# GuillaumeHolley/BloomFilterTrie

Measured on AMD Instinct MI355X. Metric: M k-mers/sec queried (presenceNode), higher is better.
Workload: dtype u64

## Files before the change

### bloomfiltertrie_amd/csrc/bft_gpu.hip

```cpp
#include <hip/hip_runtime.h>

#include <algorithm>
#include <chrono>
#include <cstring>
#include <mutex>
#include <string>
#include <vector>

#include "../../include/bft_gpu.h"
#include "bft_color_plan.h"
#include "bft_handle.h"
#include "bft_hash.h"
#include "bft_index.h"
#include "bft_run_plan.h"
#include "bft_sort.h"
#include "bft_walk.h"

#define BFT_BLOCK 256
#define BFT_ABSENT_ROW 0xFFFFFFFFu
#define BFT_MAX_GENOME_ID (1u << 24)

static thread_local std::string g_err;
int bft_fail(int code, const std::string& msg) {
    g_err = msg;
// ... 759 lines not shown
    } else if (nm == "tune") {
        if (value != 0 && h->built) {
            ENTER(h);
            CK(bft_wait_foreign_stream(h));
            HIPCK(hipStreamSynchronize(h->stream));
            CK(bft_ensure_table(h));
            CK(bft_tune_residency(h));
        }
    } else if (nm == "query_dynamic") {
        h->opt_query_dynamic = value != 0;
    } else if (nm == "query_dynamic_min") {
        h->opt_query_dynamic_min = value;
    } else if (nm == "query_chunk") {
        if (value < 1 || value > 64) return fail(BFT_GPU_E_ARG, "query_chunk must be in [1,64]");
        h->opt_query_chunk = (uint32_t)value;
    } else if (nm == "query_grid_mult") {
        if (value < 1 || value > 64) return fail(BFT_GPU_E_ARG, "query_grid_mult must be in [1,64]");
        h->opt_grid_mult = (int)value;
#if defined(BFT_PERF_PROBE)
    } else if (nm == "debug_stop") {
        h->im.debug_stop = (uint32_t)value;
#endif
    } else if (nm == "test_front_rank_mode") {
        if (value > 2) return fail(BFT_GPU_E_ARG, "test_front_rank_mode must be 0, 1 or 2");
        bft_test_front_rank_mode((int)value);
    } else if (nm == "test_front_wave_cap") {
        if (value != 0 && value != 512 && value != 1024) return fail(BFT_GPU_E_ARG, "test_front_wave_cap must be 0, 512 or 1024");
        bft_test_front_wave_cap((uint32_t)value);
    } else if (nm == "test_weak_signature") {
        if (value < 0 || value > 2) return fail(BFT_GPU_E_ARG, "test_weak_signature must be 0, 1 or 2");
// ... 108 lines not shown
```

### bloomfiltertrie_amd/csrc/bft_handle.h

```cpp
#pragma once
#include <hip/hip_runtime.h>

#include "bft_derive.h"
#include "bft_dev.h"
#include "bft_image.h"
#include "bft_ingest.h"
#include "bft_kh.h"

struct HandleScratch {
    explicit HandleScratch(const char* w) : what(w) {}
    HandleScratch(const HandleScratch&) = delete;
    HandleScratch& operator=(const HandleScratch&) = delete;
    ~HandleScratch() { if (ev) (void)hipEventDestroy(ev); }
    int acquire(hipStream_t s, bool capturing_) {
        if (used && stream != s) {
            if (capturing_) return bft_fail(BFT_GPU_E_ARG, std::string(what) + " recorded into a graph: the handle's scratch is in use on another stream");
            HIPCK(ev ? hipEventSynchronize(ev) : hipDeviceSynchronize());
            used = false;
        }
        idle = !used;
        used = true;
        stream = s;
        capturing = capturing_;
        return 0;
// ... 141 lines not shown
    uint64_t idx_sizes[9] = {0};
    int opt_wgs_per_cu = 0;
    int tuned_wgs = 0;
    int opt_probe = 0;
    int tuned_probe = 0;
    double tune_ms[3] = {0, 0, 0};
    int opt_grid_mult = 1;
    uint32_t opt_test_walk_grid = 0;
    int opt_query_dynamic = 1;
    uint64_t opt_query_dynamic_min = (uint64_t)1 << 16;
    uint32_t opt_query_chunk = 4;
    ClaimSlots claims;

    HandleScratch sq{"sequence query"};
    DevBuf sq_codes, sq_bad, sq_npos, sq_poff, sq_tmp, sq_cs, sq_tile;
    HandleScratch qc{"colour query"};
    DevBuf qc_cs, qc_tmp;
    DevBuf qc_kh;
    HandleScratch pm{"prefix query"};
    DevBuf pm_buf, pm_tmp;
    uint64_t pm_n = 0;
    HandleScratch sp{"simple paths"};
    DevBuf sp_buf, sp_tmp;
    uint64_t sp_m = 0;
    HandleScratch cc{"components"};
    DevBuf cc_buf, cc_tmp;
    uint64_t cc_m = 0, cc_sets = 0;
    HandleScratch pg{"k-mer classes"};
    DevBuf pg_buf, pg_tmp;
    uint64_t pg_m = 0, pg_sets = 0;
// ... 88 lines not shown
```

### bloomfiltertrie_amd/csrc/bft_hosttest.cpp

```cpp
#include <algorithm>
#include <cstring>
#include <string>
#include <vector>

#include "bft_hash.h"
#include "bft_index.h"
#include "bft_walk.h"
#include "bft_kh_host.h"

struct HostTrie {
    int k, L, W, B;
    std::vector<uint32_t> hashmod;
    std::vector<uint64_t> tk;
    std::vector<uint32_t> tcol, cs_off, cs_ids;
    std::vector<uint64_t> rdir, nph;
    BftKhHostTable kh;
    std::vector<uint32_t> rstart, rq, rspec;
    uint64_t rstart_plain = 0;
    BftHostIndex idx;
    BftImage im;
};

template <int W>
static void to_tform(const uint8_t* packed, uint64_t n, int B, int L, std::vector<uint64_t>& out) {
// ... 635 lines not shown
extern "C" uint64_t bft_hosttest_read_genome(void* fv, int g, uint8_t* out) {
    BftFileContent* fc = (BftFileContent*)fv;
    const std::vector<uint8_t>& v = fc->per_genome[g];
    if (out && !v.empty()) memcpy(out, v.data(), v.size());
    return v.size();
}
extern "C" void bft_hosttest_read_free(void* fv) { delete (BftFileContent*)fv; }

extern "C" int bft_hosttest_annot_encode(const uint32_t* ids, uint32_t n, uint8_t* out, uint32_t cap) {
    std::vector<uint8_t> enc;
    bft_annot_encode(ids, n, enc);
    if (enc.size() > cap) return -1;
    memcpy(out, enc.data(), enc.size());
    return (int)enc.size();
}
```

### bloomfiltertrie_amd/csrc/bft_kernels_seq.h

```cpp
#pragma once
#include "bft_kernels_seqenc.h"
#include "bft_kernels_seqwin.h"

template <int W, int BLOCK, bool STAGED, int PROBE>
__device__ __forceinline__ void seq_walk_body(const BftImage& im, const uint64_t* __restrict__ codes, const uint32_t* __restrict__ bad,
                                              const uint64_t* __restrict__ seq_off, const uint64_t* __restrict__ pos_off, const uint32_t* __restrict__ tile_seq,
                                              uint32_t n_seqs, int canonical, uint32_t* __restrict__ csout) {
    extern __shared__ __align__(16) uint8_t lds[];
    uint32_t* l_hm = (uint32_t*)lds;
    uint8_t* l_bf = lds + BFT_LDS_HM_BYTES;
    const BftNode root = im.nodes[0];
    const bool stage_root = STAGED && im.rdir == nullptr;
    const uint32_t bf_bytes = stage_root ? ((BFT_MODULO_HASH * (uint32_t)root.bf_wb + 15u) & ~15u) : 0u;
    BftCCX* l_cc = (BftCCX*)(l_bf + bf_bytes);
    {
        const uint4* g = (const uint4*)im.hashmod;
        uint4* l = (uint4*)l_hm;
        for (uint32_t i = threadIdx.x; i < BFT_LDS_HM_BYTES / 16; i += BLOCK) l[i] = g[i];
        if (stage_root) {
            const uint64_t* gb = (const uint64_t*)(im.bfT + (size_t)root.bf_off * 8);
            uint64_t* lb = (uint64_t*)l_bf;
            const uint32_t nb8 = (BFT_MODULO_HASH * (uint32_t)root.bf_wb) / 8;
            for (uint32_t i = threadIdx.x; i < nb8; i += BLOCK) lb[i] = gb[i];
            for (uint32_t i = threadIdx.x; i < root.ncc; i += BLOCK) l_cc[i] = im.ccx[root.cc_first + i];
// ... 20 lines not shown
}

template <int W, bool STAGED, int PROBE>
__global__ __launch_bounds__(1024) __attribute__((amdgpu_waves_per_eu(8, 8))) void k_seq_walk8(
    BftImage im, const uint64_t* __restrict__ codes, const uint32_t* __restrict__ bad, const uint64_t* __restrict__ seq_off, const uint64_t* __restrict__ pos_off,
    const uint32_t* __restrict__ tile_seq, uint32_t n_seqs, int canonical, uint32_t* __restrict__ csout) {
    seq_walk_body<W, 1024, STAGED, PROBE>(im, codes, bad, seq_off, pos_off, tile_seq, n_seqs, canonical, csout);
}
template <int W, bool STAGED, int PROBE>
__global__ __launch_bounds__(BFT_BLOCK6) __attribute__((amdgpu_waves_per_eu(6, 6))) void k_seq_walk6(
    BftImage im, const uint64_t* __restrict__ codes, const uint32_t* __restrict__ bad, const uint64_t* __restrict__ seq_off, const uint64_t* __restrict__ pos_off,
    const uint32_t* __restrict__ tile_seq, uint32_t n_seqs, int canonical, uint32_t* __restrict__ csout) {
    seq_walk_body<W, BFT_BLOCK6, STAGED, PROBE>(im, codes, bad, seq_off, pos_off, tile_seq, n_seqs, canonical, csout);
}

#define SEQ_TALLY_G 2048u
#define SEQ_TALLY_WAVES 4
__global__ __launch_bounds__(64 * SEQ_TALLY_WAVES) void k_seq_tally(const uint32_t* __restrict__ csin, const uint64_t* __restrict__ pos_off, uint32_t n_seqs,
                                                                   const uint32_t* __restrict__ cs_off, const void* __restrict__ cs_ids, uint32_t cs_w, uint32_t G,
                                                                   uint32_t rowbytes, double threshold, uint32_t win, uint8_t* __restrict__ out) {
    extern __shared__ uint32_t s_cnt[];
    const uint32_t lane = threadIdx.x & 63u, wave = threadIdx.x >> 6;
    uint32_t* cnt = s_cnt + (size_t)wave * win;
    for (uint64_t s = (uint64_t)blockIdx.x * SEQ_TALLY_WAVES + wave; s < n_seqs; s += (uint64_t)gridDim.x * SEQ_TALLY_WAVES) {
        const uint64_t pa = pos_off[s], m = pos_off[s + 1] - pa;
        const uint64_t minv = (uint64_t)(int64_t)ceil((double)m * threshold);
        for (uint32_t win0 = 0; win0 < G; win0 += win) {
            const uint32_t wn = min(win, G - win0);
            for (uint32_t j = lane; j < wn; j += 64) cnt[j] = 0;
            for (uint64_t base = 0; base < m; base += 128) {
                uint32_t cs[2], len[2], qa[2], qb[2];
                bool act[2];
#pragma unroll
                for (int u = 0; u < 2; u++) cs[u] = base + 64u * u + lane < m ? csin[pa + base + 64u * u + lane] : 0xFFFFFFFFu;
#pragma unroll
                for (int u = 0; u < 2; u++) {
                    const uint32_t pcs = __shfl_up(cs[u], 1);
                    const bool boundary = lane == 0 || pcs != cs[u];
                    const uint64_t bmask = __ballot(boundary);
                    const uint64_t above = lane == 63 ? 0ull : bmask >> (lane + 1);
                    len[u] = above ? (uint32_t)__builtin_ctzll(above) + 1u : 64u - lane;
                    act[u] = boundary && cs[u] != 0xFFFFFFFFu;
                    qa[u] = qb[u] = 0;
                }
#pragma unroll
                for (int u = 0; u < 2; u++)
                    if (act[u]) { qa[u] = cs_off[cs[u]]; qb[u] = cs_off[cs[u] + 1]; }
                uint32_t id[2][8];
#pragma unroll
                for (int u = 0; u < 2; u++) {
#pragma unroll
                    for (int j = 0; j < 8; j++) id[u][j] = act[u] && qb[u] > qa[u] ? bft_cs_id_at(cs_ids, cs_w, min(qa[u] + (uint32_t)j, qb[u] - 1u)) : 0u;
                }
#pragma unroll
                for (int u = 0; u < 2; u++) {
                    if (!act[u]) continue;
#pragma unroll
                    for (int j = 0; j < 8; j++)
                        if (qa[u] + (uint32_t)j < qb[u] && id[u][j] - win0 < wn) atomicAdd(&cnt[id[u][j] - win0], len[u]);
                    for (uint32_t q = qa[u] + 8u; q < qb[u]; q += 8) {
                        uint32_t more[8];
#pragma unroll
                        for (int j = 0; j < 8; j++) more[j] = bft_cs_id_at(cs_ids, cs_w, min(q + (uint32_t)j, qb[u] - 1u));
#pragma unroll
                        for (int j = 0; j < 8; j++)
                            if (q + (uint32_t)j < qb[u] && more[j] - win0 < wn) atomicAdd(&cnt[more[j] - win0], len[u]);
                    }
                }
            }
            __builtin_amdgcn_fence(__ATOMIC_ACQ_REL, "wavefront");
            for (uint32_t b = lane; b < (wn + 7u) / 8u; b += 64) {
                uint32_t v = 0;
                for (uint32_t j = 0; j < 8 && b * 8 + j < wn; j++) {
                    const uint32_t c = cnt[b * 8 + j];
                    if (c && c >= minv) v |= 1u << j;
                }
                out[s * rowbytes + win0 / 8 + b] = (uint8_t)v;
            }
            __builtin_amdgcn_fence(__ATOMIC_ACQ_REL, "wavefront");
        }
    }
}
```

### bloomfiltertrie_amd/csrc/bft_kernels_seqenc.h

```cpp
#pragma once
__device__ __forceinline__ int nt_code(char ch) {
    const uint32_t c = (uint8_t)ch, idx = (c & 0xDFu) - 0x41u;
    const uint32_t valid_mask = (1u << 0) | (1u << 2) | (1u << 6) | (1u << 19) | (1u << 20);
    const bool ok = idx < 21u && ((valid_mask >> idx) & 1u);
    return ok ? (int)(((c >> 1) ^ (c >> 2)) & 3u) : -1;
}

__global__ void k_seq_encode(const char* __restrict__ seqs, uint64_t n_chars, uint64_t n_words, uint64_t* __restrict__ codes, uint32_t* __restrict__ bad) {
    const bool aligned = ((uintptr_t)seqs & 15u) == 0;
    for (uint64_t wi = blockIdx.x * (uint64_t)blockDim.x + threadIdx.x; wi < n_words; wi += (uint64_t)gridDim.x * blockDim.x) {
        uint32_t d[8];
        if (aligned && wi * 32 + 32 <= n_chars) {
            const uint4* src = (const uint4*)(seqs + wi * 32);
            const uint4 a = src[0], b = src[1];
            d[0] = a.x; d[1] = a.y; d[2] = a.z; d[3] = a.w; d[4] = b.x; d[5] = b.y; d[6] = b.z; d[7] = b.w;
        } else {
#pragma unroll
            for (int j = 0; j < 8; j++) {
                uint32_t v = 0;
                for (int c = 0; c < 4; c++) {
                    const uint64_t at = wi * 32 + 4 * j + c;
                    v |= (uint32_t)(uint8_t)(at < n_chars ? seqs[at] : 'A') << (8 * c);
                }
                d[j] = v;
            }
// ... 39 lines not shown
```

### bloomfiltertrie_amd/csrc/bft_kh.h

```cpp
#pragma once
#include <hip/hip_runtime.h>
#include <stdint.h>

#include "bft_claims.h"
#include "bft_dev.h"
#include "bft_image.h"

#define BFT_KH_BLOCK 256
bool bft_kh_has_kernels(int W, uint32_t S);
struct BftKhScratch { DevBuf b[7]; };
int bft_kh_sort(const uint64_t* d_tk, const uint32_t* d_vals, uint64_t n, int k, int W, const BftKhGeo& g, BftKhScratch& sc, hipStream_t s);
int bft_kh_test_sort(int W, int shape, const uint32_t* keys, const void* recs, uint64_t n, unsigned b0, unsigned b1, uint32_t* ok, void* orec, hipStream_t s, uint32_t* h_dbase);
uint32_t bft_kh_test_sort_tile(int W, int shape);
int bft_kh_lay(uint64_t n, int k, int W, const BftKhGeo& g, uint64_t* d_kh, uint64_t* d_ovf_k, uint32_t* d_ovf_v, uint32_t* d_status, BftKhScratch& sc, hipStream_t s);
int bft_kh_dump(const BftImage& im, uint64_t* d_keys, uint64_t stride, uint32_t* d_vals, unsigned long long* d_cnt, hipStream_t s);
int bft_kh_query(const BftImage& im, int grid_mult, const uint8_t* d_kmers, uint64_t n, int rec, uint64_t* d_bits64, uint32_t* d_out32, BftClaimCtr d_ctr, uint32_t chunk,
                 hipStream_t s);
size_t bft_kh_colors_scratch_bytes(uint64_t n);
int bft_kh_color_rows(const BftImage& im, const uint8_t* d_kmers, uint64_t n, int rec, uint64_t* d_bits64, const uint8_t* bm, uint32_t stride, uint32_t rowbytes, uint8_t* d_out,
                      int device, hipStream_t s);
int bft_kh_colors(const BftImage& im, const uint8_t* d_kmers, uint64_t n, int rec, uint64_t* d_bits64, uint64_t* d_offsets, uint32_t* d_ids, uint64_t ids_cap, uint64_t* d_needed,
                  void* d_scratch, hipStream_t s);
int bft_kh_branching(const BftImage& im, const uint8_t* d_kmers, uint64_t n, int B, uint64_t* d_bits64, uint8_t* d_counts, BftClaimCtr d_ctr, uint32_t chunk, hipStream_t s);
int bft_kh_seq(const BftImage& im, const uint64_t* d_codes, const uint32_t* d_bad, const uint64_t* d_seq_off, const uint64_t* d_pos_off, const uint32_t* d_tile_seq,
               uint32_t n_seqs, int canonical, uint32_t* d_csout, BftClaimCtr d_ctr, uint32_t chunk, hipStream_t s);

int bft_walkh_query(const BftImage& im, const uint8_t* d_kmers, uint64_t n, int rec, uint64_t* d_bits64, uint32_t* d_rows, BftClaimCtr d_ctr, uint32_t grid_mult, uint32_t grid_cap, hipStream_t s);
```

### bloomfiltertrie_amd/csrc/bft_kh.hip

```cpp
#include <hip/hip_runtime.h>

#include <algorithm>
#include <atomic>
#include <cstring>

#include "bft_dev.h"
#include "bft_image.h"
#include "bft_kh.h"
#include "bft_claims.h"
#include "bft_walk.h"
#include "bft_kernels_load.h"
#include "bft_kernels_seqwin.h"
#include "bft_kh_dev.h"
#include "bft_scan.h"
#include "bft_rows16.h"
#include "bft_sort.h"

#define BFT_KH_MIN_CLAIM 4u
#define BFT_KH_MAX_CLAIM 64u
typedef BftClaims<BFT_KH_MIN_CLAIM> KhClaims;
template <int W, int S>
__global__ __launch_bounds__(BFT_KH_BLOCK) void k_query_kh(BftImage im, const uint8_t* __restrict__ packed, uint64_t n, int B, uint64_t* __restrict__ bits64,
                                                          uint32_t* __restrict__ out32, BftClaimCtr ctr, uint32_t chunk) {
    const uint64_t end_aligned = ((uint64_t)packed + n * (uint64_t)B) & ~3ull;
    const uint64_t nblk = (n + BFT_KH_BLOCK - 1) / BFT_KH_BLOCK, nwords = (n + 63) / 64;
    constexpr uint32_t WPB = BFT_KH_BLOCK / 64;
    __shared__ uint32_t s_next[2];
// ... 341 lines not shown
        const int branching = live && (cr > 1 || cl_ > 1);
        if (counts && live) counts[i] = (uint8_t)((cr << 4) | cl_);
        const uint64_t mask = __ballot(branching);
        if ((threadIdx.x & 63u) == 0) s_bits[(cl.blk - cl.start) * WPB + (threadIdx.x >> 6)] = mask;
        if (cl.last_of_round()) {
            __syncthreads();
            const uint64_t w0 = cl.start * WPB, w1 = min(nwords, cl.blk_end * WPB);
            if (w0 + threadIdx.x < w1) __builtin_nontemporal_store(s_bits[threadIdx.x], &bits64[w0 + threadIdx.x]);
        }
        cl.advance();
    }
    cl.done();
}

template <int W, int S>
__global__ __launch_bounds__(256) void k_seq_kh(BftImage im, const uint64_t* __restrict__ codes, const uint32_t* __restrict__ bad, const uint64_t* __restrict__ seq_off,
                                                const uint64_t* __restrict__ pos_off, const uint32_t* __restrict__ tile_seq, uint32_t n_seqs, int canonical,
                                                uint32_t* __restrict__ csout, BftClaimCtr ctr, uint32_t chunk) {
    const uint64_t P = pos_off[n_seqs];
    const uint64_t nblk = (P + 255) / 256;
    __shared__ uint32_t s_next[2];
    __shared__ uint4 s_lines[4][64 * BFT_KH_LDS_LINE];
    uint4* const wave_lines = s_lines[threadIdx.x >> 6];
    KhClaims cl(ctr, chunk, nblk, s_next);
    cl.first();
    for (; cl.blk < nblk; cl.advance()) {
        const uint64_t p = cl.blk * 256 + threadIdx.x;
        uint32_t cs = 0xFFFFFFFFu;
        uint64_t x[W], t[W];
        BftKhKey<W> key;
        key.home = 0; key.field = 0;
#pragma unroll
        for (int w = 0; w < W; w++) { key.body[w] = 0; key.bmask[w] = 0; }
        bool live = false;
        if (p < P) {
            uint32_t lo = tile_seq[p >> 6];
            while (lo + 1 < n_seqs && pos_off[lo + 1] <= p) lo++;
            if (seq_window<W>(codes, bad, seq_off[lo] + (p - pos_off[lo]), im.k, canonical, x)) {
                bft_tform_from_x<W>(x, im.k, t);
                bft_kh_key<W>(t, im.k, im.kh, key);
                live = true;
            }
        }
        kh_fetch_quad(im, key.home, live, wave_lines);
        if (live) {
            uint32_t val = 0;
            int res = kh_lds_scan<W, S>(im, wave_lines + (threadIdx.x & 63u) * BFT_KH_LDS_LINE, key, 0u, &val);
            for (uint32_t d = 1; res < 0 && d <= im.kh.maxd; d++) {
                const uint64_t* line = im.kh_lines + (key.home + d) * BFT_KH_LINE_WORDS;
                uint64_t hd[2];
                bft_kh_load_header(line, hd);
                res = bft_kh_scan<W, S>(im, line, hd, key, d, &val);
            }
            if (res < 0 && im.kh_ovf_n) res = bft_kh_overflow_find<W>(im, t, &val) ? 1 : 0;
            if (res > 0) cs = val;
        }
        if (p < P) csout[p] = cs;
    }
    cl.done();
}

template <int W>
struct __attribute__((packed, aligned(4))) KhRec {
    uint64_t t[W];
    uint32_t v;
};
template <int W>
struct KhSortIn {
    const uint64_t* tk;
    const uint32_t* vals;
    int k;
    BftKhGeo g;
    __device__ __forceinline__ uint32_t key(uint32_t i) const {
        uint64_t t[W];
// ... 297 lines not shown
    KH_DISPATCH(im.W, (int)im.kh.S, (kh_color_rows_launch<KW, KS>(im, d_kmers, n, rec, d_bits64, bm, stride, rowbytes, plan.tile_rows, plan.div_m, plan.div_l, d_out, device, s)));
    HIPCK(hipGetLastError());
    return 0;
}

int bft_kh_branching(const BftImage& im, const uint8_t* d_kmers, uint64_t n, int B, uint64_t* d_bits64, uint8_t* d_counts, BftClaimCtr d_ctr, uint32_t chunk, hipStream_t s) {
    const dim3 block(BFT_KH_BLOCK);
    chunk = std::max(1u, std::min(chunk, BFT_KH_BR_MAX_CLAIM));
    const dim3 grid = kh_round_grid(n, chunk, 1, d_ctr.p != nullptr);
    KH_DISPATCH(im.W, (int)im.kh.S, hipLaunchKernelGGL((k_branching_kh<KW, KS>), grid, block, 0, s, im, d_kmers, n, B, d_bits64, d_counts, d_ctr, chunk));
    HIPCK(hipGetLastError());
    return 0;
}

int bft_kh_seq(const BftImage& im, const uint64_t* d_codes, const uint32_t* d_bad, const uint64_t* d_seq_off, const uint64_t* d_pos_off, const uint32_t* d_tile_seq,
               uint32_t n_seqs, int canonical, uint32_t* d_csout, BftClaimCtr d_ctr, uint32_t chunk, hipStream_t s) {
    const dim3 grid(256 * 8), block(256);
    chunk = std::max(1u, std::min(chunk, BFT_KH_MAX_CLAIM));
    KH_DISPATCH(im.W, (int)im.kh.S,
                hipLaunchKernelGGL((k_seq_kh<KW, KS>), grid, block, 0, s, im, d_codes, d_bad, d_seq_off, d_pos_off, d_tile_seq, n_seqs, canonical, d_csout, d_ctr, chunk));
    HIPCK(hipGetLastError());
    return 0;
}
```

### bloomfiltertrie_amd/csrc/bft_query.hip

```cpp
#include <hip/hip_runtime.h>

#include <algorithm>
#include <atomic>
#include <cstring>
#include <initializer_list>
#include <type_traits>
#include <vector>

#include "bft_handle.h"
#include "bft_scan.h"
#include "bft_walk.h"

#define BFT_BLOCK 256
#define BFT_ABSENT_ROW 0xFFFFFFFFu

#include "bft_kernels_query.h"
#include "bft_kernels_seq.h"
#include "bft_kernels_color.h"

void ClaimSlots::ensure() {
    if (ctr || failed) return;
    if (hipMalloc((void**)&ctr, KH_CTR_SLOTS * 8) != hipSuccess || hipMemset(ctr, 0, KH_CTR_SLOTS * 8) != hipSuccess ||
        hipDeviceSynchronize() != hipSuccess) {
        (void)hipGetLastError();
// ... 588 lines not shown
    DevBuf dk, db, dr, dout;
    CK(dk.alloc(mc * h->B));
    CK(db.alloc(((mc + 63) / 64) * 8));
    CK(dr.alloc(mc * 4));
    CK(dout.alloc(mc * rowbytes));
    for (uint64_t a = 0; a < n; a += chunk) {
        const uint64_t m = std::min(chunk, n - a);
        CK(query_rows(h, kmers + a * h->B, m, dk, db, dr, present_bits ? present_bits + a / 8 : nullptr));
        CK(launch_color_rows(h, dr.as<uint32_t>(), m, rowbytes, dout.as<uint8_t>(), h->stream));
        HIPCK(hipMemcpyAsync(rows + a * rowbytes, dout.p, m * rowbytes, hipMemcpyDeviceToHost, h->stream));
        HIPCK(hipStreamSynchronize(h->stream));
    }
    return BFT_GPU_OK;
}

static int launch_seq_lookups(bft_gpu* h, const BftImage& image, uint32_t ns, int canonical, const uint64_t* d_soff, uint64_t units, hipStream_t s) {
    if (image.kh_lines != nullptr) {
        const ClaimSlots::Claim claim = h->claims.take(s, claims_wanted(h, h->opt_query_dynamic_min), units);
        CK(bft_kh_seq(image, h->sq_codes.as<uint64_t>(), h->sq_bad.as<uint32_t>(), d_soff, h->sq_poff.as<uint64_t>(), h->sq_tile.as<uint32_t>(), ns, canonical,
                      h->sq_cs.as<uint32_t>(), claim.ctr, h->opt_query_chunk, s));
        h->claims.launched(claim.slot, s);
        return 0;
    }
    BftImage im = image;
    im.emit_cs = 1;
    return walk_dispatch<false>(h, false, [&](auto w, auto staged, auto probe) {
        constexpr int W = decltype(w)::value, PROBE = decltype(probe)::value;
        constexpr bool STAGED = decltype(staged)::value;
        static std::atomic<uint64_t> lds_allowed{0};
        auto launch = [&](auto kernel, const WalkShape& sh) {
            CK(allow_walk_lds(lds_allowed, h->device, {(const void*)kernel}));
            hipLaunchKernelGGL(kernel, dim3(512), dim3(sh.block), sh.lds, s, im, h->sq_codes.as<uint64_t>(), h->sq_bad.as<uint32_t>(), d_soff, h->sq_poff.as<uint64_t>(),
                               h->sq_tile.as<uint32_t>(), ns, canonical, h->sq_cs.as<uint32_t>());
            HIPCK(hipGetLastError());
            return 0;
// ... 8 lines not shown
    const uint32_t G = h->im.nb_genomes, rowbytes = (G + 7) / 8;
    if (rowbytes == 0 || n_seqs == 0) return 0;
    CK(h->sq.acquire(s, bft_stream_capturing(s)));
    auto need = [&](DevBuf& b, size_t bytes) { return h->sq.grow(b, bytes, bytes / 8); };
    const uint64_t chunk = 1ull << 30;
    const uint64_t cmax = std::min(chunk, n_seqs);
    const uint64_t n_cw = (total_chars + 31) / 32;
    const size_t scan_bytes = bft_scan::scratch_bytes(cmax + 1);
    CK(need(h->sq_codes, (n_cw + BFT_MAX_W + 2) * 8));
    CK(need(h->sq_bad, (n_cw + BFT_MAX_W + 2) * 4));
    CK(need(h->sq_npos, (cmax + 1) * 8));
    CK(need(h->sq_poff, (cmax + 1) * 8));
    CK(need(h->sq_tmp, scan_bytes));
    CK(need(h->sq_tile, (total_chars / 64 + 2) * 4));
    CK(need(h->sq_cs, (total_chars + 64) * 4));
    CK(bft_zero_async(h->sq_codes.as<uint64_t>() + n_cw, (BFT_MAX_W + 2) * 8, s));
    CK(bft_zero_async(h->sq_bad.as<uint32_t>() + n_cw, (BFT_MAX_W + 2) * 4, s));
    if (n_cw)
        CK(bft_timed_launch(h, s, [&] {
            hipLaunchKernelGGL(k_seq_encode, dim3(bft_grid_for((n_cw + 255) / 256)), dim3(256), 0, s, d_seqs, total_chars, n_cw, h->sq_codes.as<uint64_t>(),
                               h->sq_bad.as<uint32_t>());
            HIPCK(hipGetLastError());
            return 0;
        }));
    for (uint64_t a = 0; a < n_seqs; a += chunk) {
        const uint64_t ns = std::min(chunk, n_seqs - a);
        const uint64_t* soff = d_seq_off + a;
        CK(bft_timed_launch(h, s, [&] {
            hipLaunchKernelGGL(k_seq_plan, dim3(bft_grid_for((ns + 256) / 256)), dim3(256), 0, s, soff, ns, h->k, h->sq_npos.as<uint64_t>());
            CK(bft_scan::exclusive_sum_ptr<uint64_t>(h->sq_npos.as<uint64_t>(), h->sq_poff.as<uint64_t>(), ns + 1, s, h->sq_tmp));
            hipLaunchKernelGGL(k_seq_tiles, dim3(256 * 4), dim3(256), 0, s, h->sq_poff.as<uint64_t>(), (uint32_t)ns, h->sq_tile.as<uint32_t>());
            HIPCK(hipGetLastError());
            return 0;
        }));
        CK(bft_timed_launch(h, s, [&] { return launch_seq_lookups(h, h->im, (uint32_t)ns, canonical, soff, total_chars / 256 + 2, s); }));
        const uint32_t win = std::min<uint32_t>(SEQ_TALLY_G, (G + 63u) & ~63u);
        CK(bft_timed_launch(h, s, [&] {
            hipLaunchKernelGGL(k_seq_tally, dim3((unsigned)std::min<uint64_t>((ns + SEQ_TALLY_WAVES - 1) / SEQ_TALLY_WAVES, 256ull * 16)), dim3(64 * SEQ_TALLY_WAVES),
                               (size_t)SEQ_TALLY_WAVES * win * 4, s, h->sq_cs.as<uint32_t>(), h->sq_poff.as<uint64_t>(), (uint32_t)ns, h->im.cs_off, h->im.cs_ids, h->im.cs_w, G,
                               rowbytes, threshold, win, d_rows + a * rowbytes);
            HIPCK(hipGetLastError());
            return 0;
        }));
    }
    h->sq.release();
    return 0;
}

extern "C" int bft_gpu_query_sequences_dev(bft_gpu* h, const void* d_seqs, const void* d_seq_off, uint64_t n_seqs, uint64_t total_chars, double threshold,
                                           int canonical, void* d_rows, void* hip_stream) {
    if (!h || ((!d_seqs || !d_seq_off || !d_rows) && n_seqs)) return bft_fail(BFT_GPU_E_ARG, "NULL argument");
    if (!(threshold > 0) || threshold > 1) return bft_fail(BFT_GPU_E_ARG, "the threshold must be in (0, 1] (reference src/bft.c:1246-1247)");
    ENTER(h);
    CK(bft_ensure_built(h, false));
    hipStream_t s = hip_stream ? (hipStream_t)hip_stream : h->stream;
// ... 59 lines not shown
```

Baseline: 52920.

## Fuse sequence k-mer lookups with colour tally for short sequences

Adds a fused k_seq_rows_kh kernel that, per group of positions, does the hash-table lookups into an LDS slice and immediately tallies colour sets into output rows. This avoids writing and re-reading the per-position colour-set buffer for short sequences. Long sequences fall back to the old lookup-then-tally kernels, which now skip short ones and exit early when no long sequences exist. The encode kernel also zeroes the slack words itself, replacing two memset launches. The change only affects sequence queries, not the measured presenceNode k-mer path.

Measured after the change: 52840. No clear change (-0.1%).

```diff
diff --git a/bloomfiltertrie_amd/csrc/bft_gpu.hip b/bloomfiltertrie_amd/csrc/bft_gpu.hip
--- a/bloomfiltertrie_amd/csrc/bft_gpu.hip
+++ b/bloomfiltertrie_amd/csrc/bft_gpu.hip
@@ -797,6 +797,9 @@
     } else if (nm == "query_chunk") {
         if (value < 1 || value > 64) return fail(BFT_GPU_E_ARG, "query_chunk must be in [1,64]");
         h->opt_query_chunk = (uint32_t)value;
+    } else if (nm == "seq_fused") {
+        if (value != 0 && value != 1) return fail(BFT_GPU_E_ARG, "seq_fused must be 0 or 1");
+        h->opt_seq_fused = (int)value;
     } else if (nm == "query_grid_mult") {
         if (value < 1 || value > 64) return fail(BFT_GPU_E_ARG, "query_grid_mult must be in [1,64]");
         h->opt_grid_mult = (int)value;
diff --git a/bloomfiltertrie_amd/csrc/bft_handle.h b/bloomfiltertrie_amd/csrc/bft_handle.h
--- a/bloomfiltertrie_amd/csrc/bft_handle.h
+++ b/bloomfiltertrie_amd/csrc/bft_handle.h
@@ -179,6 +179,8 @@
 
     HandleScratch sq{"sequence query"};
     DevBuf sq_codes, sq_bad, sq_npos, sq_poff, sq_tmp, sq_cs, sq_tile;
+    DevBuf sq_nlong;
+    int opt_seq_fused = 1;
     HandleScratch qc{"colour query"};
     DevBuf qc_cs, qc_tmp;
     DevBuf qc_kh;
diff --git a/bloomfiltertrie_amd/csrc/bft_hosttest.cpp b/bloomfiltertrie_amd/csrc/bft_hosttest.cpp
--- a/bloomfiltertrie_amd/csrc/bft_hosttest.cpp
+++ b/bloomfiltertrie_amd/csrc/bft_hosttest.cpp
@@ -7,6 +7,7 @@
 #include "bft_index.h"
 #include "bft_walk.h"
 #include "bft_kh_host.h"
+#include "bft_seq_plan.h"
 
 struct HostTrie {
     int k, L, W, B;
@@ -673,3 +674,21 @@
     memcpy(out, enc.data(), enc.size());
     return (int)enc.size();
 }
+
+extern "C" int64_t bft_hosttest_seq_plan(const uint64_t* pos_off, uint32_t n_seqs, uint64_t total_chars, uint32_t genomes, uint32_t* first_out, uint64_t cap, uint64_t* consts) {
+    const uint64_t P = pos_off[n_seqs], ntiles = (P + 63) / 64, groups = bft_seq_groups(P);
+    consts[0] = BFT_SEQ_Q; consts[1] = BFT_SEQ_C; consts[2] = BFT_SEQ_LMAX; consts[3] = BFT_SEQ_WAVES; consts[4] = groups;
+    consts[5] = bft_seq_units_bound(total_chars); consts[6] = bft_seq_lds_bytes(bft_seq_win(genomes)); consts[7] = bft_seq_win(genomes);
+    if (cap < groups + 1) return -1;
+    std::vector<uint32_t> tile_seq(ntiles + 1, 0xFFFFFFFFu);
+    for (uint64_t t = 0; t < ntiles; t++) {
+        uint32_t lo = 0, hi = n_seqs;
+        while (hi - lo > 1) {
+            const uint32_t mid = (lo + hi) >> 1;
+            if (pos_off[mid] <= t * 64) lo = mid; else hi = mid;
+        }
+        tile_seq[t] = lo;
+    }
+    for (uint64_t g = 0; g <= groups; g++) first_out[g] = bft_seq_group_first(pos_off, tile_seq.data(), n_seqs, P, g);
+    return (int64_t)groups;
+}
diff --git a/bloomfiltertrie_amd/csrc/bft_kernels_seq.h b/bloomfiltertrie_amd/csrc/bft_kernels_seq.h
--- a/bloomfiltertrie_amd/csrc/bft_kernels_seq.h
+++ b/bloomfiltertrie_amd/csrc/bft_kernels_seq.h
@@ -1,6 +1,8 @@
 #pragma once
 #include "bft_kernels_seqenc.h"
 #include "bft_kernels_seqwin.h"
+#include "bft_kernels_seqtally.h"
+#include "bft_seq_plan.h"
 
 template <int W, int BLOCK, bool STAGED, int PROBE>
 __device__ __forceinline__ void seq_walk_body(const BftImage& im, const uint64_t* __restrict__ codes, const uint32_t* __restrict__ bad,
@@ -58,70 +60,17 @@
     seq_walk_body<W, BFT_BLOCK6, STAGED, PROBE>(im, codes, bad, seq_off, pos_off, tile_seq, n_seqs, canonical, csout);
 }
 
-#define SEQ_TALLY_G 2048u
 #define SEQ_TALLY_WAVES 4
 __global__ __launch_bounds__(64 * SEQ_TALLY_WAVES) void k_seq_tally(const uint32_t* __restrict__ csin, const uint64_t* __restrict__ pos_off, uint32_t n_seqs,
                                                                    const uint32_t* __restrict__ cs_off, const void* __restrict__ cs_ids, uint32_t cs_w, uint32_t G,
-                                                                   uint32_t rowbytes, double threshold, uint32_t win, uint8_t* __restrict__ out) {
+                                                                   uint32_t rowbytes, double threshold, uint32_t win, uint8_t* __restrict__ out, const uint32_t* __restrict__ n_long) {
     extern __shared__ uint32_t s_cnt[];
+    if (n_long && *n_long == 0) return;
     const uint32_t lane = threadIdx.x & 63u, wave = threadIdx.x >> 6;
     uint32_t* cnt = s_cnt + (size_t)wave * win;
     for (uint64_t s = (uint64_t)blockIdx.x * SEQ_TALLY_WAVES + wave; s < n_seqs; s += (uint64_t)gridDim.x * SEQ_TALLY_WAVES) {
         const uint64_t pa = pos_off[s], m = pos_off[s + 1] - pa;
-        const uint64_t minv = (uint64_t)(int64_t)ceil((double)m * threshold);
-        for (uint32_t win0 = 0; win0 < G; win0 += win) {
-            const uint32_t wn = min(win, G - win0);
-            for (uint32_t j = lane; j < wn; j += 64) cnt[j] = 0;
-            for (uint64_t base = 0; base < m; base += 128) {
-                uint32_t cs[2], len[2], qa[2], qb[2];
-                bool act[2];
-#pragma unroll
-                for (int u = 0; u < 2; u++) cs[u] = base + 64u * u + lane < m ? csin[pa + base + 64u * u + lane] : 0xFFFFFFFFu;
-#pragma unroll
-                for (int u = 0; u < 2; u++) {
-                    const uint32_t pcs = __shfl_up(cs[u], 1);
-                    const bool boundary = lane == 0 || pcs != cs[u];
-                    const uint64_t bmask = __ballot(boundary);
-                    const uint64_t above = lane == 63 ? 0ull : bmask >> (lane + 1);
-                    len[u] = above ? (uint32_t)__builtin_ctzll(above) + 1u : 64u - lane;
-                    act[u] = boundary && cs[u] != 0xFFFFFFFFu;
-                    qa[u] = qb[u] = 0;
-                }
-#pragma unroll
-                for (int u = 0; u < 2; u++)
-                    if (act[u]) { qa[u] = cs_off[cs[u]]; qb[u] = cs_off[cs[u] + 1]; }
-                uint32_t id[2][8];
-#pragma unroll
-                for (int u = 0; u < 2; u++) {
-#pragma unroll
-                    for (int j = 0; j < 8; j++) id[u][j] = act[u] && qb[u] > qa[u] ? bft_cs_id_at(cs_ids, cs_w, min(qa[u] + (uint32_t)j, qb[u] - 1u)) : 0u;
-                }
-#pragma unroll
-                for (int u = 0; u < 2; u++) {
-                    if (!act[u]) continue;
-#pragma unroll
-                    for (int j = 0; j < 8; j++)
-                        if (qa[u] + (uint32_t)j < qb[u] && id[u][j] - win0 < wn) atomicAdd(&cnt[id[u][j] - win0], len[u]);
-                    for (uint32_t q = qa[u] + 8u; q < qb[u]; q += 8) {
-                        uint32_t more[8];
-#pragma unroll
-                        for (int j = 0; j < 8; j++) more[j] = bft_cs_id_at(cs_ids, cs_w, min(q + (uint32_t)j, qb[u] - 1u));
-#pragma unroll
-                        for (int j = 0; j < 8; j++)
-                            if (q + (uint32_t)j < qb[u] && more[j] - win0 < wn) atomicAdd(&cnt[more[j] - win0], len[u]);
-                    }
-                }
-            }
-            __builtin_amdgcn_fence(__ATOMIC_ACQ_REL, "wavefront");
-            for (uint32_t b = lane; b < (wn + 7u) / 8u; b += 64) {
-                uint32_t v = 0;
-                for (uint32_t j = 0; j < 8 && b * 8 + j < wn; j++) {
-                    const uint32_t c = cnt[b * 8 + j];
-                    if (c && c >= minv) v |= 1u << j;
-                }
-                out[s * rowbytes + win0 / 8 + b] = (uint8_t)v;
-            }
-            __builtin_amdgcn_fence(__ATOMIC_ACQ_REL, "wavefront");
-        }
+        if (n_long && m <= BFT_SEQ_LMAX) continue;
+        seq_tally_row([&](uint64_t j) { return csin[pa + j]; }, m, cnt, lane, cs_off, cs_ids, cs_w, G, threshold, win, out + s * rowbytes);
     }
 }
diff --git a/bloomfiltertrie_amd/csrc/bft_kernels_seqenc.h b/bloomfiltertrie_amd/csrc/bft_kernels_seqenc.h
--- a/bloomfiltertrie_amd/csrc/bft_kernels_seqenc.h
+++ b/bloomfiltertrie_amd/csrc/bft_kernels_seqenc.h
@@ -6,9 +6,15 @@
     return ok ? (int)(((c >> 1) ^ (c >> 2)) & 3u) : -1;
 }
 
+#define BFT_SEQ_SLACK_WORDS (BFT_MAX_W + 2)
 __global__ void k_seq_encode(const char* __restrict__ seqs, uint64_t n_chars, uint64_t n_words, uint64_t* __restrict__ codes, uint32_t* __restrict__ bad) {
     const bool aligned = ((uintptr_t)seqs & 15u) == 0;
-    for (uint64_t wi = blockIdx.x * (uint64_t)blockDim.x + threadIdx.x; wi < n_words; wi += (uint64_t)gridDim.x * blockDim.x) {
+    for (uint64_t wi = blockIdx.x * (uint64_t)blockDim.x + threadIdx.x; wi < n_words + BFT_SEQ_SLACK_WORDS; wi += (uint64_t)gridDim.x * blockDim.x) {
+        if (wi >= n_words) {
+            codes[wi] = 0;
+            bad[wi] = 0;
+            continue;
+        }
         uint32_t d[8];
         if (aligned && wi * 32 + 32 <= n_chars) {
             const uint4* src = (const uint4*)(seqs + wi * 32);
diff --git a/bloomfiltertrie_amd/csrc/bft_kernels_seqtally.h b/bloomfiltertrie_amd/csrc/bft_kernels_seqtally.h
--- /dev/null
+++ b/bloomfiltertrie_amd/csrc/bft_kernels_seqtally.h
@@ -0,0 +1,64 @@
+#pragma once
+#include "bft_walk.h"
+
+#define SEQ_TALLY_G 2048u
+
+template <class CsAt>
+__device__ __forceinline__ void seq_tally_row(CsAt cs_at, uint64_t m, uint32_t* cnt, uint32_t lane, const uint32_t* __restrict__ cs_off, const void* __restrict__ cs_ids,
+                                              uint32_t cs_w, uint32_t G, double threshold, uint32_t win, uint8_t* __restrict__ out_row) {
+    const uint64_t minv = (uint64_t)(int64_t)ceil((double)m * threshold);
+    for (uint32_t win0 = 0; win0 < G; win0 += win) {
+        const uint32_t wn = min(win, G - win0);
+        for (uint32_t j = lane; j < wn; j += 64) cnt[j] = 0;
+        for (uint64_t base = 0; base < m; base += 128) {
+            uint32_t cs[2], len[2], qa[2], qb[2];
+            bool act[2];
+#pragma unroll
+            for (int u = 0; u < 2; u++) cs[u] = base + 64u * u + lane < m ? cs_at(base + 64u * u + lane) : 0xFFFFFFFFu;
+#pragma unroll
+            for (int u = 0; u < 2; u++) {
+                const uint32_t pcs = __shfl_up(cs[u], 1);
+                const bool boundary = lane == 0 || pcs != cs[u];
+                const uint64_t bmask = __ballot(boundary);
+                const uint64_t above = lane == 63 ? 0ull : bmask >> (lane + 1);
+                len[u] = above ? (uint32_t)__builtin_ctzll(above) + 1u : 64u - lane;
+                act[u] = boundary && cs[u] != 0xFFFFFFFFu;
+                qa[u] = qb[u] = 0;
+            }
+#pragma unroll
+            for (int u = 0; u < 2; u++)
+                if (act[u]) { qa[u] = cs_off[cs[u]]; qb[u] = cs_off[cs[u] + 1]; }
+            uint32_t id[2][8];
+#pragma unroll
+            for (int u = 0; u < 2; u++) {
+#pragma unroll
+                for (int j = 0; j < 8; j++) id[u][j] = act[u] && qb[u] > qa[u] ? bft_cs_id_at(cs_ids, cs_w, min(qa[u] + (uint32_t)j, qb[u] - 1u)) : 0u;
+            }
+#pragma unroll
+            for (int u = 0; u < 2; u++) {
+                if (!act[u]) continue;
+#pragma unroll
+                for (int j = 0; j < 8; j++)
+                    if (qa[u] + (uint32_t)j < qb[u] && id[u][j] - win0 < wn) atomicAdd(&cnt[id[u][j] - win0], len[u]);
+                for (uint32_t q = qa[u] + 8u; q < qb[u]; q += 8) {
+                    uint32_t more[8];
+#pragma unroll
+                    for (int j = 0; j < 8; j++) more[j] = bft_cs_id_at(cs_ids, cs_w, min(q + (uint32_t)j, qb[u] - 1u));
+#pragma unroll
+                    for (int j = 0; j < 8; j++)
+                        if (q + (uint32_t)j < qb[u] && more[j] - win0 < wn) atomicAdd(&cnt[more[j] - win0], len[u]);
+                }
+            }
+        }
+        __builtin_amdgcn_fence(__ATOMIC_ACQ_REL, "wavefront");
+        for (uint32_t b = lane; b < (wn + 7u) / 8u; b += 64) {
+            uint32_t v = 0;
+            for (uint32_t j = 0; j < 8 && b * 8 + j < wn; j++) {
+                const uint32_t c = cnt[b * 8 + j];
+                if (c && c >= minv) v |= 1u << j;
+            }
+            out_row[win0 / 8 + b] = (uint8_t)v;
+        }
+        __builtin_amdgcn_fence(__ATOMIC_ACQ_REL, "wavefront");
+    }
+}
diff --git a/bloomfiltertrie_amd/csrc/bft_kh.h b/bloomfiltertrie_amd/csrc/bft_kh.h
--- a/bloomfiltertrie_amd/csrc/bft_kh.h
+++ b/bloomfiltertrie_amd/csrc/bft_kh.h
@@ -23,6 +23,9 @@
                   void* d_scratch, hipStream_t s);
 int bft_kh_branching(const BftImage& im, const uint8_t* d_kmers, uint64_t n, int B, uint64_t* d_bits64, uint8_t* d_counts, BftClaimCtr d_ctr, uint32_t chunk, hipStream_t s);
 int bft_kh_seq(const BftImage& im, const uint64_t* d_codes, const uint32_t* d_bad, const uint64_t* d_seq_off, const uint64_t* d_pos_off, const uint32_t* d_tile_seq,
-               uint32_t n_seqs, int canonical, uint32_t* d_csout, BftClaimCtr d_ctr, uint32_t chunk, hipStream_t s);
+               uint32_t n_seqs, int canonical, uint32_t* d_csout, const uint32_t* d_n_long, BftClaimCtr d_ctr, uint32_t chunk, hipStream_t s);
+int bft_kh_seq_rows(const BftImage& im, const uint64_t* d_codes, const uint32_t* d_bad, const uint64_t* d_seq_off, const uint64_t* d_pos_off, const uint32_t* d_tile_seq,
+                    uint32_t n_seqs, int canonical, double threshold, uint32_t win, uint8_t* d_rows, uint32_t* d_n_long, uint64_t units, BftClaimCtr d_ctr, uint32_t chunk, int device,
+                    hipStream_t s);
 
 int bft_walkh_query(const BftImage& im, const uint8_t* d_kmers, uint64_t n, int rec, uint64_t* d_bits64, uint32_t* d_rows, BftClaimCtr d_ctr, uint32_t grid_mult, uint32_t grid_cap, hipStream_t s);
diff --git a/bloomfiltertrie_amd/csrc/bft_kh.hip b/bloomfiltertrie_amd/csrc/bft_kh.hip
--- a/bloomfiltertrie_amd/csrc/bft_kh.hip
+++ b/bloomfiltertrie_amd/csrc/bft_kh.hip
@@ -11,6 +11,8 @@
 #include "bft_walk.h"
 #include "bft_kernels_load.h"
 #include "bft_kernels_seqwin.h"
+#include "bft_kernels_seqtally.h"
+#include "bft_seq_plan.h"
 #include "bft_kh_dev.h"
 #include "bft_scan.h"
 #include "bft_rows16.h"
@@ -382,9 +384,29 @@
 }
 
 template <int W, int S>
+__device__ __forceinline__ uint32_t kh_seq_lookup(const BftImage& im, const BftKhKey<W>& key, const uint64_t* t, bool live, uint4* wave_lines) {
+    uint32_t cs = 0xFFFFFFFFu;
+    kh_fetch_quad(im, key.home, live, wave_lines);
+    if (live) {
+        uint32_t val = 0;
+        int res = kh_lds_scan<W, S>(im, wave_lines + (threadIdx.x & 63u) * BFT_KH_LDS_LINE, key, 0u, &val);
+        for (uint32_t d = 1; res < 0 && d <= im.kh.maxd; d++) {
+            const uint64_t* line = im.kh_lines + (key.home + d) * BFT_KH_LINE_WORDS;
+            uint64_t hd[2];
+            bft_kh_load_header(line, hd);
+            res = bft_kh_scan<W, S>(im, line, hd, key, d, &val);
+        }
+        if (res < 0 && im.kh_ovf_n) res = bft_kh_overflow_find<W>(im, t, &val) ? 1 : 0;
+        if (res > 0) cs = val;
+    }
+    return cs;
+}
+
+template <int W, int S>
 __global__ __launch_bounds__(256) void k_seq_kh(BftImage im, const uint64_t* __restrict__ codes, const uint32_t* __restrict__ bad, const uint64_t* __restrict__ seq_off,
                                                 const uint64_t* __restrict__ pos_off, const uint32_t* __restrict__ tile_seq, uint32_t n_seqs, int canonical,
-                                                uint32_t* __restrict__ csout, BftClaimCtr ctr, uint32_t chunk) {
+                                                uint32_t* __restrict__ csout, const uint32_t* __restrict__ n_long, BftClaimCtr ctr, uint32_t chunk) {
+    if (n_long && *n_long == 0) return;
     const uint64_t P = pos_off[n_seqs];
     const uint64_t nblk = (P + 255) / 256;
     __shared__ uint32_t s_next[2];
@@ -394,38 +416,92 @@
     cl.first();
     for (; cl.blk < nblk; cl.advance()) {
         const uint64_t p = cl.blk * 256 + threadIdx.x;
-        uint32_t cs = 0xFFFFFFFFu;
         uint64_t x[W], t[W];
         BftKhKey<W> key;
         key.home = 0; key.field = 0;
 #pragma unroll
         for (int w = 0; w < W; w++) { key.body[w] = 0; key.bmask[w] = 0; }
-        bool live = false;
+        bool live = false, mine = p < P;
         if (p < P) {
             uint32_t lo = tile_seq[p >> 6];
             while (lo + 1 < n_seqs && pos_off[lo + 1] <= p) lo++;
-            if (seq_window<W>(codes, bad, seq_off[lo] + (p - pos_off[lo]), im.k, canonical, x)) {
+            const uint64_t pa = pos_off[lo];
+            if (n_long && pos_off[lo + 1] - pa <= BFT_SEQ_LMAX) mine = false;
+            if (mine && seq_window<W>(codes, bad, seq_off[lo] + (p - pa), im.k, canonical, x)) {
                 bft_tform_from_x<W>(x, im.k, t);
                 bft_kh_key<W>(t, im.k, im.kh, key);
                 live = true;
             }
         }
-        kh_fetch_quad(im, key.home, live, wave_lines);
-        if (live) {
-            uint32_t val = 0;
-            int res = kh_lds_scan<W, S>(im, wave_lines + (threadIdx.x & 63u) * BFT_KH_LDS_LINE, key, 0u, &val);
-            for (uint32_t d = 1; res < 0 && d <= im.kh.maxd; d++) {
-                const uint64_t* line = im.kh_lines + (key.home + d) * BFT_KH_LINE_WORDS;
-                uint64_t hd[2];
-                bft_kh_load_header(line, hd);
-                res = bft_kh_scan<W, S>(im, line, hd, key, d, &val);
-            }
-            if (res < 0 && im.kh_ovf_n) res = bft_kh_overflow_find<W>(im, t, &val) ? 1 : 0;
-            if (res > 0) cs = val;
-        }
-        if (p < P) csout[p] = cs;
+        const uint32_t cs = kh_seq_lookup<W, S>(im, key, t, live, wave_lines);
+        if (mine) csout[p] = cs;
     }
     cl.done();
+}
+
+template <int W, int S>
+__global__ __launch_bounds__(64 * BFT_SEQ_WAVES) void k_seq_rows_kh(BftImage im, const uint64_t* __restrict__ codes, const uint32_t* __restrict__ bad,
+                                                                   const uint64_t* __restrict__ seq_off, const uint64_t* __restrict__ pos_off,
+                                                                   const uint32_t* __restrict__ tile_seq, uint32_t n_seqs, int canonical, double threshold, uint32_t win,
+                                                                   uint8_t* __restrict__ out, uint32_t* __restrict__ n_long, BftClaimCtr ctr, uint32_t chunk) {
+    __shared__ uint32_t s_next[2];
+    __shared__ uint4 s_lines[BFT_SEQ_WAVES][64 * BFT_KH_LDS_LINE];
+    __shared__ uint32_t s_cs_all[BFT_SEQ_WAVES][BFT_SEQ_C];
+    static_assert(BFT_SEQ_WIN_MAX * 4u <= 64u * BFT_KH_LDS_LINE * 16u, "the counters fit the wavefront's lines");
+    const uint32_t lane = threadIdx.x & 63u, wave = (uint32_t)__builtin_amdgcn_readfirstlane((int)(threadIdx.x >> 6));
+    uint4* const wave_lines = s_lines[wave];
+    uint32_t* const s_cs = s_cs_all[wave];
+    uint32_t* const cnt = reinterpret_cast<uint32_t*>(wave_lines);
+    const uint32_t G = im.nb_genomes, rowbytes = (G + 7u) / 8u;
+    const uint64_t P = pos_off[n_seqs];
+    const uint64_t ngroups = bft_seq_groups(P), nblk = (ngroups + BFT_SEQ_WAVES - 1u) / BFT_SEQ_WAVES;
+    uint32_t longs = 0;
+    KhClaims cl(ctr, chunk, nblk, s_next);
+    cl.first();
+    for (; cl.blk < nblk; cl.advance()) {
+        const uint64_t g = cl.blk * BFT_SEQ_WAVES + wave;
+        if (g >= ngroups) continue;
+        const uint32_t s0 = bft_seq_group_first(pos_off, tile_seq, n_seqs, P, g);
+        uint32_t s1 = bft_seq_group_first(pos_off, tile_seq, n_seqs, P, g + 1u);
+        if (s0 >= s1) continue;
+        if (pos_off[s1] - pos_off[s1 - 1u] > BFT_SEQ_LMAX) {
+            s1--;
+            longs++;
+        }
+        const uint64_t pa = pos_off[s0], pe = pos_off[s1];
+        const uint32_t span = (uint32_t)(pe - pa);
+        __builtin_amdgcn_wave_barrier();
+        uint32_t lo = s0;
+#pragma unroll 1
+        for (uint32_t j0 = 0; j0 < span; j0 += 64u) {
+            const uint64_t p = pa + j0 + lane;
+            uint64_t x[W], t[W];
+            BftKhKey<W> key;
+            key.home = 0; key.field = 0;
+#pragma unroll
+            for (int w = 0; w < W; w++) { key.body[w] = 0; key.bmask[w] = 0; }
+            bool live = false;
+            if (p < pe) {
+                while (lo + 1u < s1 && pos_off[lo + 1u] <= p) lo++;
+                if (seq_window<W>(codes, bad, seq_off[lo] + (p - pos_off[lo]), im.k, canonical, x)) {
+                    bft_tform_from_x<W>(x, im.k, t);
+                    bft_kh_key<W>(t, im.k, im.kh, key);
+                    live = true;
+                }
+            }
+            s_cs[j0 + lane] = kh_seq_lookup<W, S>(im, key, t, live, wave_lines);
+        }
+        __builtin_amdgcn_fence(__ATOMIC_RELEASE, "wavefront");
+        __builtin_amdgcn_wave_barrier();
+        __builtin_amdgcn_fence(__ATOMIC_ACQUIRE, "wavefront");
+        for (uint32_t s = s0; s < s1; s++) {
+            const uint64_t a = pos_off[s], m = pos_off[s + 1u] - a;
+            const uint32_t* const cs_s = s_cs + (uint32_t)(a - pa);
+            seq_tally_row([&](uint64_t j) { return cs_s[j]; }, m, cnt, lane, im.cs_off, im.cs_ids, im.cs_w, G, threshold, win, out + (uint64_t)s * rowbytes);
+        }
+    }
+    cl.done();
+    if (lane == 0 && longs) atomicAdd(n_long, longs);
 }
 
 template <int W>
@@ -753,11 +829,41 @@
 }
 
 int bft_kh_seq(const BftImage& im, const uint64_t* d_codes, const uint32_t* d_bad, const uint64_t* d_seq_off, const uint64_t* d_pos_off, const uint32_t* d_tile_seq,
-               uint32_t n_seqs, int canonical, uint32_t* d_csout, BftClaimCtr d_ctr, uint32_t chunk, hipStream_t s) {
+               uint32_t n_seqs, int canonical, uint32_t* d_csout, const uint32_t* d_n_long, BftClaimCtr d_ctr, uint32_t chunk, hipStream_t s) {
     const dim3 grid(256 * 8), block(256);
     chunk = std::max(1u, std::min(chunk, BFT_KH_MAX_CLAIM));
     KH_DISPATCH(im.W, (int)im.kh.S,
-                hipLaunchKernelGGL((k_seq_kh<KW, KS>), grid, block, 0, s, im, d_codes, d_bad, d_seq_off, d_pos_off, d_tile_seq, n_seqs, canonical, d_csout, d_ctr, chunk));
+                hipLaunchKernelGGL((k_seq_kh<KW, KS>), grid, block, 0, s, im, d_codes, d_bad, d_seq_off, d_pos_off, d_tile_seq, n_seqs, canonical, d_csout, d_n_long, d_ctr, chunk));
     HIPCK(hipGetLastError());
     return 0;
 }
+
+template <int W, int S>
+static int kh_seq_rows_launch(const BftImage& im, const uint64_t* d_codes, const uint32_t* d_bad, const uint64_t* d_seq_off, const uint64_t* d_pos_off, const uint32_t* d_tile_seq,
+                              uint32_t n_seqs, int canonical, double threshold, uint32_t win, uint8_t* d_rows, uint32_t* d_n_long, uint64_t units, BftClaimCtr d_ctr, uint32_t chunk,
+                              int device, hipStream_t s) {
+    static std::atomic<int> resident_dev[64];
+    std::atomic<int>& res = resident_dev[device & 63];
+    int r = res.load(std::memory_order_relaxed);
+    if (!r) {
+        int per_cu = 0, cus = 0;
+        if (hipOccupancyMaxActiveBlocksPerMultiprocessor(&per_cu, k_seq_rows_kh<W, S>, 64 * BFT_SEQ_WAVES, 0) != hipSuccess || per_cu < 1) { per_cu = 4; (void)hipGetLastError(); }
+        if (hipDeviceGetAttribute(&cus, hipDeviceAttributeMultiprocessorCount, device) != hipSuccess || cus < 1) { cus = 256; (void)hipGetLastError(); }
+        r = per_cu * cus;
+        res.store(r, std::memory_order_relaxed);
+    }
+    const dim3 grid((unsigned)std::max<uint64_t>(1, std::min<uint64_t>((units + chunk - 1) / chunk, (uint64_t)r)));
+    hipLaunchKernelGGL((k_seq_rows_kh<W, S>), grid, dim3(64 * BFT_SEQ_WAVES), 0, s, im, d_codes, d_bad, d_seq_off, d_pos_off, d_tile_seq, n_seqs, canonical, threshold, win, d_rows,
+                       d_n_long, d_ctr, chunk);
+    return 0;
+}
+
+int bft_kh_seq_rows(const BftImage& im, const uint64_t* d_codes, const uint32_t* d_bad, const uint64_t* d_seq_off, const uint64_t* d_pos_off, const uint32_t* d_tile_seq,
+                    uint32_t n_seqs, int canonical, double threshold, uint32_t win, uint8_t* d_rows, uint32_t* d_n_long, uint64_t units, BftClaimCtr d_ctr, uint32_t chunk, int device,
+                    hipStream_t s) {
+    chunk = std::max(1u, std::min(chunk, BFT_KH_MAX_CLAIM));
+    KH_DISPATCH(im.W, (int)im.kh.S,
+                CK((kh_seq_rows_launch<KW, KS>(im, d_codes, d_bad, d_seq_off, d_pos_off, d_tile_seq, n_seqs, canonical, threshold, win, d_rows, d_n_long, units, d_ctr, chunk, device, s))));
+    HIPCK(hipGetLastError());
+    return 0;
+}
diff --git a/bloomfiltertrie_amd/csrc/bft_query.hip b/bloomfiltertrie_amd/csrc/bft_query.hip
--- a/bloomfiltertrie_amd/csrc/bft_query.hip
+++ b/bloomfiltertrie_amd/csrc/bft_query.hip
@@ -626,11 +626,11 @@
     return BFT_GPU_OK;
 }
 
-static int launch_seq_lookups(bft_gpu* h, const BftImage& image, uint32_t ns, int canonical, const uint64_t* d_soff, uint64_t units, hipStream_t s) {
+static int launch_seq_lookups(bft_gpu* h, const BftImage& image, uint32_t ns, int canonical, const uint64_t* d_soff, uint64_t units, hipStream_t s, bool long_only = false) {
     if (image.kh_lines != nullptr) {
         const ClaimSlots::Claim claim = h->claims.take(s, claims_wanted(h, h->opt_query_dynamic_min), units);
         CK(bft_kh_seq(image, h->sq_codes.as<uint64_t>(), h->sq_bad.as<uint32_t>(), d_soff, h->sq_poff.as<uint64_t>(), h->sq_tile.as<uint32_t>(), ns, canonical,
-                      h->sq_cs.as<uint32_t>(), claim.ctr, h->opt_query_chunk, s));
+                      h->sq_cs.as<uint32_t>(), long_only ? h->sq_nlong.as<uint32_t>() : nullptr, claim.ctr, h->opt_query_chunk, s));
         h->claims.launched(claim.slot, s);
         return 0;
     }
@@ -669,8 +669,8 @@
     CK(need(h->sq_tmp, scan_bytes));
     CK(need(h->sq_tile, (total_chars / 64 + 2) * 4));
     CK(need(h->sq_cs, (total_chars + 64) * 4));
-    CK(bft_zero_async(h->sq_codes.as<uint64_t>() + n_cw, (BFT_MAX_W + 2) * 8, s));
-    CK(bft_zero_async(h->sq_bad.as<uint32_t>() + n_cw, (BFT_MAX_W + 2) * 4, s));
+    const bool fused = h->opt_seq_fused && h->im.kh_lines != nullptr;
+    if (fused) CK(need(h->sq_nlong, 8));
     if (n_cw)
         CK(bft_timed_launch(h, s, [&] {
             hipLaunchKernelGGL(k_seq_encode, dim3(bft_grid_for((n_cw + 255) / 256)), dim3(256), 0, s, d_seqs, total_chars, n_cw, h->sq_codes.as<uint64_t>(),
@@ -688,12 +688,24 @@
             HIPCK(hipGetLastError());
             return 0;
         }));
-        CK(bft_timed_launch(h, s, [&] { return launch_seq_lookups(h, h->im, (uint32_t)ns, canonical, soff, total_chars / 256 + 2, s); }));
+        const uint32_t* const n_long = fused ? h->sq_nlong.as<uint32_t>() : nullptr;
+        if (fused) {
+            CK(bft_timed_launch(h, s, [&] {
+                CK(bft_zero_async(h->sq_nlong.p, 4, s));
+                const uint64_t units = bft_seq_units_bound(total_chars);
+                const ClaimSlots::Claim claim = h->claims.take(s, claims_wanted(h, h->opt_query_dynamic_min), units);
+                CK(bft_kh_seq_rows(h->im, h->sq_codes.as<uint64_t>(), h->sq_bad.as<uint32_t>(), soff, h->sq_poff.as<uint64_t>(), h->sq_tile.as<uint32_t>(), (uint32_t)ns, canonical,
+                                   threshold, bft_seq_win(G), d_rows + a * rowbytes, h->sq_nlong.as<uint32_t>(), units, claim.ctr, h->opt_query_chunk, h->device, s));
+                h->claims.launched(claim.slot, s);
+                return 0;
+            }));
+        }
+        CK(bft_timed_launch(h, s, [&] { return launch_seq_lookups(h, h->im, (uint32_t)ns, canonical, soff, total_chars / 256 + 2, s, fused); }));
         const uint32_t win = std::min<uint32_t>(SEQ_TALLY_G, (G + 63u) & ~63u);
         CK(bft_timed_launch(h, s, [&] {
             hipLaunchKernelGGL(k_seq_tally, dim3((unsigned)std::min<uint64_t>((ns + SEQ_TALLY_WAVES - 1) / SEQ_TALLY_WAVES, 256ull * 16)), dim3(64 * SEQ_TALLY_WAVES),
                                (size_t)SEQ_TALLY_WAVES * win * 4, s, h->sq_cs.as<uint32_t>(), h->sq_poff.as<uint64_t>(), (uint32_t)ns, h->im.cs_off, h->im.cs_ids, h->im.cs_w, G,
-                               rowbytes, threshold, win, d_rows + a * rowbytes);
+                               rowbytes, threshold, win, d_rows + a * rowbytes, n_long);
             HIPCK(hipGetLastError());
             return 0;
         }));
diff --git a/bloomfiltertrie_amd/csrc/bft_seq_plan.h b/bloomfiltertrie_amd/csrc/bft_seq_plan.h
--- /dev/null
+++ b/bloomfiltertrie_amd/csrc/bft_seq_plan.h
@@ -0,0 +1,36 @@
+#pragma once
+#include <stdint.h>
+
+#if defined(__HIPCC__)
+#define BFT_SEQ_HD __host__ __device__ __forceinline__
+#else
+#define BFT_SEQ_HD static inline
+#endif
+
+#ifndef BFT_SEQ_Q
+#define BFT_SEQ_Q 128u
+#endif
+#ifndef BFT_SEQ_C
+#define BFT_SEQ_C 384u
+#endif
+#define BFT_SEQ_LMAX (BFT_SEQ_C - BFT_SEQ_Q + 1u)
+#define BFT_SEQ_WAVES 4u
+static_assert(BFT_SEQ_Q % 64u == 0 && BFT_SEQ_C % 64u == 0, "groups start at a tile of k_seq_tiles; the lookups fill the slice 64 at a time");
+static_assert(BFT_SEQ_LMAX + 1u >= BFT_SEQ_Q, "a long sequence is the last of its group");
+static_assert(BFT_SEQ_Q - 1u + BFT_SEQ_LMAX <= BFT_SEQ_C, "a group's short sequences fit the slice");
+
+BFT_SEQ_HD uint64_t bft_seq_groups(uint64_t P) { return P / BFT_SEQ_Q + 1u; }
+BFT_SEQ_HD uint64_t bft_seq_units_bound(uint64_t total_chars) { return (bft_seq_groups(total_chars) + BFT_SEQ_WAVES - 1u) / BFT_SEQ_WAVES; }
+
+BFT_SEQ_HD uint32_t bft_seq_group_first(const uint64_t* pos_off, const uint32_t* tile_seq, uint32_t n_seqs, uint64_t P, uint64_t g) {
+    const uint64_t p0 = g * BFT_SEQ_Q;
+    if (p0 > P) return n_seqs;
+    uint32_t lo = p0 < P ? tile_seq[p0 / 64u] : n_seqs;
+    if (pos_off[lo] < p0) return lo + 1u;
+    while (lo > 0 && pos_off[lo - 1u] == p0) lo--;
+    return lo;
+}
+
+#define BFT_SEQ_WIN_MAX 1280u
+BFT_SEQ_HD uint32_t bft_seq_win(uint32_t G) { return ((G + 63u) & ~63u) < BFT_SEQ_WIN_MAX ? ((G + 63u) & ~63u) : BFT_SEQ_WIN_MAX; }
+BFT_SEQ_HD uint32_t bft_seq_lds_bytes(uint32_t win) { return (void)win, BFT_SEQ_WAVES * 64u * 80u + BFT_SEQ_WAVES * BFT_SEQ_C * 4u + 8u; }
```
